# abcqmars/audio-visual-sepatation-in-visual-agnostic-situtation

Measured on AMD Instinct MI355X. Metric: mixtures/sec (train step, 2-src MUSIC shape), higher is better.
Workload: dtype f32; 1 GPU; full HIP path, AV train step: 2-source mix, batch 64/GPU (BASELINE configs[2] shape), 65535-sample waveforms -> HIP STFT 1022/256 -> 256x256 log-freq tiles, 3x224^2 frames/source, unet7+hidsep(sig)+resnet18dilated, BCE, SGD; f32 arithmetic; visual trunk on this library (no MIOpen kernel in the step); global_batch=64, parallelism=dp1

## Files before the change

### audio-visual-sepatation-in-visual-agnostic-situtation_amd/csrc/ops.hip

```cpp
#include "common.h"
#include "warp_coords.h"
#include <string.h>
#include <stdio.h>

__global__ __launch_bounds__(256) void channel_stats_kernel(const float* __restrict__ x, int N, int C, int HW,
                                                            double* __restrict__ stats) {
  const int c = blockIdx.x;
  const long long total = (long long)N * HW;
  const long long per = (total + gridDim.y - 1) / gridDim.y;
  const long long beg = per * blockIdx.y, end = min(total, beg + per);
  float s = 0.f, q = 0.f;
  double ds = 0.0, dq = 0.0;
  int cnt = 0;
  for (long long i = beg + threadIdx.x; i < end; i += 256) {
    int n = (int)(i / HW), hw = (int)(i % HW);
    float v = x[((long long)n * C + c) * HW + hw];
    s += v;
    q += v * v;
    if (++cnt == 64) { ds += s; dq += q; s = q = 0.f; cnt = 0; }
  }
  ds += s;
  dq += q;
  block_stats_add(ds, dq, c, C, stats);
}
// ... 115 lines not shown

enum { FORM_VEC4, FORM_SCALAR };
static bool plane_grid_ok(int N, int C, long long HW) {
  return N > 0 && N <= 65535 && C > 0 && C <= 65535 && HW > 0 && HW <= 0x7fffffffLL;
}
static GluePlan bn_bwd_apply_plan(int N, int C, long long HW) {
  if (!plane_grid_ok(N, C, HW)) return glue_refused();
  int gx = min(cdiv(HW, 1024), 64);
  return GluePlan{(HW & 3) == 0 ? FORM_VEC4 : FORM_SCALAR, dim3(gx, C, N)};
}
extern "C" int avsep_bn_bwd_apply(const float* dz, const float* y, const float* pqr, int32_t N, int32_t C, int32_t HW,
                                  float* dy, avsep_stream_t stream) {
  const GluePlan pl = bn_bwd_apply_plan(N, C, HW);
  if (!dz || !y || !pqr || !dy || pl.refused()) return AVSEP_ERR_ARG;
  hipLaunchKernelGGL(bn_bwd_apply_kernel, pl.grid, dim3(256), 0, (hipStream_t)stream, dz, y, pqr, C, HW, dy);
  AVSEP_LAUNCH_CHECK();
  return AVSEP_OK;
}

__global__ __launch_bounds__(256) void affine_act_kernel(const float* __restrict__ y, const float* __restrict__ scale,
                                                         const float* __restrict__ shift,
                                                         const float* __restrict__ res, const float* __restrict__ rscale,
                                                         const float* __restrict__ rshift, int act, int C, int HW,
                                                         float* __restrict__ z) {
  const int c = blockIdx.y, n = blockIdx.z;
  const float sc = scale ? scale[c] : 1.f, sh = shift ? shift[c] : 0.f;
  const float rs = rscale ? rscale[c] : 1.f, rh = rscale ? rshift[c] : 0.f;
  const long long base = ((long long)n * C + c) * HW;
  if ((HW & 3) == 0) {
    const float slope = act_slope(act);
// ... 344 lines not shown
      atomicAdd(&bstats1[cs], sh2[0] + sh2[1] + sh2[2] + sh2[3]);
      atomicAdd(&bstats1[a.C1 + cs], sh2[4] + sh2[5] + sh2[6] + sh2[7]);
    }
  }
}

static CatArgs make_cat(const avsep_cat_desc* d) {
  CatArgs a{};
  a.N = d->N; a.C0 = d->C0; a.C1 = d->C1; a.H = d->H; a.W = d->W; a.b0 = d->bcast0; a.b1 = d->bcast1;
  a.x0 = d->x0; a.x1 = d->x1; a.sc0 = d->scale0; a.sh0 = d->shift0; a.sc1 = d->scale1; a.sh1 = d->shift1;
  a.rh = (float)(d->H - 1) / (float)(2 * d->H - 1);
  a.rw = (float)(d->W - 1) / (float)(2 * d->W - 1);
  return a;
}
static bool cat_ok(const avsep_cat_desc* d) {
  return d && d->C0 > 0 && d->C1 >= 0 && d->x0 && (d->C1 == 0 || d->x1);
}

static int up2x_pair_lw(int H, int W, bool bcast) {
  if (bcast || W < 4 || W > 128 || (W & (W - 1)) || H < 2) return -1;
  int lw = 0;
  while ((2 << lw) < W) ++lw;
  return lw;
}
enum { UP2X_FWD_PAIR, UP2X_FWD_4, UP2X_FWD_GENERIC };
static GluePlan relu_up2x_fwd_plan(int N, int C, int H, int W, bool bcast) {
  if (N <= 0 || C <= 0 || H <= 0 || W <= 0) return glue_refused();
  const long long planes = (long long)N * C;
  if (planes > 0x7fffffffLL || 2 * H > 65535) return glue_refused();
  const int plw = up2x_pair_lw(H, W, bcast);
  if (plw >= 0 && planes <= 32768LL * 65535) {
// ... 135 lines not shown
    }
    const unsigned gy = (unsigned)(planes < 32768 ? planes : 32768), gz = (unsigned)cdiv(planes, gy);
    return GluePlan{UP2X_BWD_SWEEP, dim3(cdiv((long long)tp, 256), gy, gz), {plw, 0}};
  }
  if (C > 65535) return glue_refused();
  int tilesX = cdiv(W, UB_TW), tiles = tilesX * cdiv(H, UB_TH);
  int chunks = min(cdiv(4096, C * tiles), N);
  if (chunks < 1) chunks = 1;
  return GluePlan{UP2X_BWD_TILE, dim3(tiles, C, chunks), {tilesX, 0}};
}
extern "C" int avsep_relu_up2x_bwd(const avsep_cat_desc* d, const float* dout, float* g0, float* g1,
                                   const float* mean1, const float* invstd1, double* bstats1, int32_t acc0,
                                   avsep_stream_t stream) {
  if (!cat_ok(d) || !dout) return AVSEP_ERR_ARG;
  if (bstats1 && (!mean1 || !invstd1 || d->bcast1 || !g1)) return AVSEP_ERR_ARG;
  const GluePlan pl = relu_up2x_bwd_plan(d->N, d->C0 + d->C1, d->H, d->W, d->bcast0 || d->bcast1);
  if (pl.refused()) return AVSEP_ERR_ARG;
  CatArgs a = make_cat(d);
  switch (pl.form) {
    case UP2X_BWD_SWEEP_PLANES:
      hipLaunchKernelGGL(relu_up2x_bwd_sweep_kernel<true>, pl.grid, dim3(256), 0, (hipStream_t)stream, a, dout, g0, g1, mean1,
                         invstd1, bstats1, acc0, pl.arg[0], pl.arg[1]);
      break;
    case UP2X_BWD_SWEEP:
      hipLaunchKernelGGL(relu_up2x_bwd_sweep_kernel<false>, pl.grid, dim3(256), 0, (hipStream_t)stream, a, dout, g0, g1, mean1,
                         invstd1, bstats1, acc0, pl.arg[0], 0);
      break;
    case UP2X_BWD_TILE:
      hipLaunchKernelGGL(relu_up2x_bwd_kernel, pl.grid, dim3(256), 0, (hipStream_t)stream, a, dout, g0, g1, mean1, invstd1,
                         bstats1, acc0, pl.arg[0]);
// ... 728 lines not shown
    atomicAdd(&sums[r * 3 + 2], sh[8] + sh[9] + sh[10] + sh[11]);
  }
}
extern "C" int avsep_sdr_sums(const float* est, const float* ref, int32_t R, int32_t L, int64_t est_stride,
                              int64_t ref_stride, double* sums, avsep_stream_t stream) {
  if (!est || !ref || !sums || R <= 0 || R > 65535 || L <= 0) return AVSEP_ERR_ARG;
  hipLaunchKernelGGL(sdr_sums_kernel, dim3(min(cdiv(L, 2048), 64), R), dim3(256), 0, (hipStream_t)stream, est, ref, L,
                     (long long)est_stride, (long long)ref_stride, sums);
  AVSEP_LAUNCH_CHECK();
  return AVSEP_OK;
}

static const GluePlanRow ops_glue_rows[] = {
    {"channel_stats", {"chunks"}, [](int N, int C, int H, int W, int) { return channel_stats_plan(N, C, (long long)H * W); }},
    {"bn_bwd_apply", {"vec4", "scalar"}, [](int N, int C, int H, int W, int) { return bn_bwd_apply_plan(N, C, (long long)H * W); }},
    {"affine_act", {"vec4", "scalar"}, [](int N, int C, int H, int W, int) { return affine_act_plan(N, C, (long long)H * W); }},
    {"affine_act_bwd", {"v4", "v1"}, [](int N, int C, int H, int W, int) { return affine_act_bwd_plan(N, C, (long long)H * W); }},
    {"relu_up2x_fwd", {"pair", "fwd4", "generic"}, [](int N, int C, int H, int W, int aux) { return relu_up2x_fwd_plan(N, C, H, W, aux != 0); }},
    {"relu_up2x_bwd", {"sweep,planes", "sweep", "tile"}, [](int N, int C, int H, int W, int aux) { return relu_up2x_bwd_plan(N, C, H, W, aux != 0); }},
    {"maxpool_fwd", {"fwd4", "generic"}, [](int N, int C, int H, int W, int) { return maxpool_fwd_plan(C, (long long)N * C, H, W); }},
    {"maxpool_bwd", {"gather"}, [](int N, int C, int H, int W, int) { return maxpool_bwd_plan((long long)N * C, H, W); }},
    {"maxpool_bn_relu_bwd_stats", {"plane"}, [](int N, int C, int H, int W, int) { return maxpool_bn_relu_bwd_stats_plan(N, C, H, W); }},
    {"maxpool_bn_relu_bwd_apply", {"apply4", "pair", "apply1"}, [](int N, int C, int H, int W, int) { return maxpool_bn_relu_bwd_apply_plan(N, C, H, W); }},
    {"space_to_depth2", {"planes"}, [](int N, int C, int H, int W, int Cp) { return space_to_depth2_plan(N, C, H, W, Cp); }},
    {"temporal_mean_fwd", {"flat"}, [](int B, int C, int H, int W, int T) { return temporal_mean_plan(B, T, (long long)C * H * W, false); }},
    {"temporal_mean_bwd", {"flat"}, [](int B, int C, int H, int W, int T) { return temporal_mean_plan(B, T, (long long)C * H * W, true); }},
    {"sgd", {"flat"}, [](int N, int C, int H, int W, int) { return flat_plan((long long)N * C * ((long long)H * W), 16384); }},
};

extern "C" int avsep_glue_plan(const char* op, int32_t N, int32_t C, int32_t H, int32_t W, int32_t aux, char* form, size_t cap,
// ... 28 lines not shown
```

### audio-visual-sepatation-in-visual-agnostic-situtation_amd/kernels.py

```python
import ctypes as C
import os

import numpy as np
import torch

from . import lib
from .lib import ConvDesc, CatDesc, call, ptr


def _f32(shape, like):
    return torch.empty(shape, dtype=torch.float32, device=like.device)


FMT_F32, FMT_B16 = 0, 1


def is_b16(t):
    return t is not None and t.dtype == torch.bfloat16


def fmt_of(t):
    return FMT_B16 if is_b16(t) else FMT_F32


# ... 482 lines not shown
    N, Cc, H, W = dims(y)
    if to_b16_out and not is_b16(y) and not is_b16(dz) and b16_ok(Cc):
        dst = _b16((N, Cc, H, W), y)
        call("avsep_bn_bwd_apply_to_b16", ptr(dz), ptr(y), ptr(pqr), N, Cc, H * W, ptr(dst))
        return dst
    (dz,) = _same_fmt(y, dz)
    dst = torch.empty_like(y) if fresh else (dz if out is None else out)
    _drop_twin(dst)
    if is_b16(y):
        call("avsep_b16_bn_bwd_apply", ptr(dz), ptr(y), ptr(pqr), N, Cc, H * W, ptr(dst))
    else:
        call("avsep_bn_bwd_apply", ptr(dz), ptr(y), ptr(pqr), N, Cc, H * W, ptr(dst))
    return dst


def affine_act(y, scale, shift, residual, act, res_scale=None, res_shift=None):
    N, Cc, H, W = dims(y)
    z = torch.empty_like(y)
    (residual,) = _same_fmt(y, residual)
    if is_b16(y):
        call("avsep_b16_affine_act", ptr(y), ptr(scale), ptr(shift), ptr(residual), ptr(res_scale), ptr(res_shift), act, N, Cc,
             H * W, ptr(z))
    else:
        call("avsep_affine_act", ptr(y), ptr(scale), ptr(shift), ptr(residual), ptr(res_scale), ptr(res_shift), act, N, Cc,
             H * W, ptr(z))
    return z


def affine_act_bwd_(dz, y, scale, shift, residual, add, mean, invstd, act, bstats, res_scale=None, res_shift=None,
                    out=None, dz2=None, stats_only=False):
# ... 5 lines not shown
             ptr(res_shift), ptr(add), ptr(mean), ptr(invstd), act, N, Cc, H * W, None, ptr(bstats))
        return dz
    _drop_twin(dst)
    if is_b16(y):
        call("avsep_b16_affine_act_bwd", ptr(dz), ptr(dz2), ptr(y), ptr(scale), ptr(shift), ptr(residual), ptr(res_scale),
             ptr(res_shift), ptr(add), ptr(mean), ptr(invstd), act, N, Cc, H * W, ptr(dst), ptr(bstats))
    else:
        call("avsep_affine_act_bwd", ptr(dz), ptr(dz2), ptr(y), ptr(scale), ptr(shift), ptr(residual), ptr(res_scale), ptr(res_shift),
             ptr(add), ptr(mean), ptr(invstd), act, N, Cc, H * W, ptr(dst), ptr(bstats))
    return dst


class Cat:

    def __init__(self, x0, x1, sc0=None, sh0=None, sc1=None, sh1=None, bcast0=False, hw=None):
        self.b16 = (not bcast0 and x1 is not None and (is_b16(x0) or is_b16(x1)) and b16_ok(channels(x0))
                    and b16_ok(channels(x1)))
        if self.b16:
            x0, x1 = to_b16(x0), to_b16(x1)
        else:
            x0, x1 = to_f32(x0), to_f32(x1)
        N, C0 = (x0.shape[0], x0.shape[1]) if bcast0 else dims(x0)[:2]
        C1 = channels(x1) if x1 is not None else 0
        H, W = hw if hw is not None else (dims(x1)[2:] if x1 is not None else dims(x0)[2:])
        self.shape = (N, C0, C1, H, W)
        self.keep = (x0, x1, sc0, sh0, sc1, sh1)
        d = CatDesc()
        d.N, d.C0, d.C1, d.H, d.W, d.bcast0, d.bcast1 = N, C0, C1, H, W, int(bcast0), 0
        d.x0, d.x1 = ptr(x0), ptr(x1)
        d.scale0, d.shift0, d.scale1, d.shift1 = ptr(sc0), ptr(sh0), ptr(sc1), ptr(sh1)
        self.d, self.ref, self.like, self.bcast0 = d, C.byref(d), (x1 if x1 is not None else x0), bcast0

    def fwd(self):
        N, C0, C1, H, W = self.shape
        x0, x1, sc0, sh0, sc1, sh1 = self.keep
        if self.b16:
            out = _b16((N, C0 + C1, 2 * H, 2 * W), self.like)
# ... 4 lines not shown
        return out

    def bwd(self, dout, mean1=None, invstd1=None, bstats1=None, g0_acc=None):
        N, C0, C1, H, W = self.shape
        x0, x1, sc0, sh0, sc1, sh1 = self.keep
        if self.b16:
            dout = to_b16(dout)
            g0 = g0_acc if g0_acc is not None else _b16((N, C0, H, W), self.like)
            assert is_b16(g0), "accumulating into an fp32 skip gradient from a B16 decoder level"
            _drop_twin(g0)
            g1 = _b16((N, C1, H, W), self.like)
            call("avsep_b16_relu_up2x_bwd", ptr(x0), ptr(x1), ptr(sc0), ptr(sh0), ptr(sc1), ptr(sh1), N, C0, C1, H, W, ptr(dout),
                 ptr(g0), ptr(g1), ptr(mean1), ptr(invstd1), ptr(bstats1), int(g0_acc is not None))
            return g0, g1
        dout = to_f32(dout)
        g0 = g0_acc if g0_acc is not None else _f32((N, C0) if self.bcast0 else (N, C0, H, W), self.like)
        assert not is_b16(g0)
        _drop_twin(g0)
        g1 = _f32((N, C1, H, W), self.like) if C1 else None
        call("avsep_relu_up2x_bwd", self.ref, ptr(dout), ptr(g0), ptr(g1), ptr(mean1), ptr(invstd1),
             ptr(bstats1), int(g0_acc is not None))
        return g0, g1


def prepare(mag_mix, mags, log_freq, weighted, binary, fout=256):
    lib.require_gpu(mag_mix)
    S, B, _, Fin, T = mags.shape
    Fo = fout if log_freq else Fin
    mix_w, logm, weight = (_f32((B, 1, Fo, T), mag_mix) for _ in range(3))
    mags_w, gt = _f32((S, B, 1, Fo, T), mag_mix), _f32((S, B, 1, Fo, T), mag_mix)
    call("avsep_prepare", ptr(mag_mix), ptr(mags), S, B, Fin, T, Fo, int(bool(log_freq)), int(bool(weighted)),
         int(bool(binary)), ptr(mix_w), ptr(mags_w), ptr(logm), ptr(weight), ptr(gt))
    return mix_w, mags_w, logm, weight, gt
# ... 785 lines not shown
```

### audio-visual-sepatation-in-visual-agnostic-situtation_amd/lib.py

```python
import ctypes as C
import os

import torch

_HERE = os.path.dirname(os.path.abspath(__file__))
LIB_PATH = os.path.join(_HERE, "libavsep_gfx950.so")

ACT_NONE, ACT_RELU, ACT_LRELU02, ACT_SIGMOID, ACT_TANH, ACT_SOFTMAX2 = range(6)
ACT_BY_NAME = {"no": ACT_NONE, "relu": ACT_RELU, "sigmoid": ACT_SIGMOID, "tanh": ACT_TANH,
               "softmax": ACT_SOFTMAX2}
LOSS_BY_NAME = {"bce": 0, "l1": 1, "l2": 2}
ATT_BY_NAME = {"cos": 0, "sig": 1}
ALGO_NO = {"winograd": 1, "winograd_wgrad": 2, "flat": 4, "misc_patch": 8, "bf16_kernels": 16, "smallci_wgrad": 32, "winograd4": 64}


class AvsepError(RuntimeError):
    pass


class ConvDesc(C.Structure):
    _fields_ = [(n, C.c_int32) for n in
                "N Cin H W Cout Ho Wo KH KW stride pad dil C0 act0 act1 up2x prec plan_n xfmt yfmt dyfmt dxfmt algo tune".split()] + \
               [(n, C.c_void_p) for n in "x0 x1 scale0 shift0 scale1 shift1".split()]

# ... 56 lines not shown
    "avsep_conv_kernel_name": (C.c_char_p, [_CD, _I, _I]),
    "avsep_conv_kernel_variant": (C.c_int, [_CD, _I, _I, C.c_char_p, _Z]),
    "avsep_space_to_depth2": (C.c_int, [_P, _I, _I, _I, _I, _I, _P, _P]),
    "avsep_maxpool_bn_relu_bwd_stats": (C.c_int, [_P, _P, _P, _P, _P, _P, _P, _I, _I, _I, _I, _P, _P]),
    "avsep_maxpool_bn_relu_bwd_apply": (C.c_int, [_P, _P, _P, _P, _P, _P, _I, _I, _I, _I, _P, _P]),
    "avsep_attmodel_infer_fwd": (C.c_int, [_P, _P, _I, _I, _I, _I, _I, _P, _P, _P, _P]),
    "avsep_attmodel_infer_bwd": (C.c_int, [_P, _P, _P, _P, _P, _P, _I, _I, _I, _I, _I, _P, _P, _P]),
    "avsep_conv2d_dgrad_up2x_workspace_bytes": (_Z, [_CD]),
    "avsep_conv2d_dgrad_up2x": (C.c_int, [_CD, _P, _P, _P, _P, _P, _P, _P, _I, _P, _Z, _P]),
    "avsep_conv2d_wgrad_workspace_bytes": (_Z, [_CD]),
    "avsep_conv2d_wgrad": (C.c_int, [_CD, _P, _P, _P, _P, _Z, _P]),
    "avsep_channel_stats": (C.c_int, [_P, _I, _I, _I, _P, _P]),
    "avsep_bn_finalize": (C.c_int, [_P, _D, _P, _P, _P, _P, _F, _F, _I, _I, _P, _P, _P, _P, _P, _I, _P]),
    "avsep_bn_bwd_coeffs": (C.c_int, [_P, _D, _P, _P, _P, _I, _P, _P, _P, _P]),
    "avsep_bn_bwd_apply": (C.c_int, [_P, _P, _P, _I, _I, _I, _P, _P]),
    "avsep_affine_act": (C.c_int, [_P, _P, _P, _P, _P, _P, _I, _I, _I, _I, _P, _P]),
    "avsep_affine_act_bwd": (C.c_int, [_P, _P, _P, _P, _P, _P, _P, _P, _P, _P, _P, _I, _I, _I, _I, _P, _P, _P]),
    "avsep_relu_up2x_fwd": (C.c_int, [_KD, _P, _P]),
    "avsep_relu_up2x_bwd": (C.c_int, [_KD, _P, _P, _P, _P, _P, _P, _I, _P]),
    "avsep_prepare": (C.c_int, [_P, _P, _I, _I, _I, _I, _I, _I, _I, _I, _P, _P, _P, _P, _P, _P]),
    "avsep_warp": (C.c_int, [_P, _I, _I, _I, _I, _I, _I, _P, _P]),
    "avsep_window_prepare": (C.c_int, [_P, _I, _I, _P, _I, _I, _I, _P, _P, _P]),
    "avsep_window_agreement": (C.c_int, [_P, _P, _I, _I, _I, _I, _P, _P]),
    "avsep_mask_stitch": (C.c_int, [_P, _P, _P, _P, _I, _I, _I, _I, _I, _I, _I, _I, _F, _P, _P, _P]),
    "avsep_window_reduce": (C.c_int, [_P, _P, _I, _I, C.c_int64, _I, _P, _P]),
    "avsep_mwf_workspace_bytes": (_Z, [_I, _I, _I, _I]),
    "avsep_mwf_cov": (C.c_int, [_P, _P, _I, _I, _I, _I, _I, _P, _P, _Z, _P]),
    "avsep_mwf_apply": (C.c_int, [_P, _P, _P, _P, _I, _I, _I, _I, _F, _P, _P, _P]),
    "avsep_mwf_tv_workspace_bytes": (_Z, [_I, _I, _I, _I, _I]),
    "avsep_mwf_cov_tv": (C.c_int, [_P, _P, _I, _I, _I, _I, _I, _I, _P, _P, _Z, _P]),
# ... 128 lines not shown
```

### audio-visual-sepatation-in-visual-agnostic-situtation_amd/models/audio_net.py

```python
import os

import torch
import torch.nn as nn

from .. import kernels as K
from .. import lib
from ..lib import ACT_LRELU02, ACT_NONE, ACT_RELU
from . import fusion_net

BN_EPS, BN_MOMENTUM = 1e-5, 0.1


class _Slots(nn.Module):
    def put(self, idx, mod):
        self.add_module(str(idx), mod)
        return mod

    def at(self, idx):
        return getattr(self, str(idx))


class Conv2dParams(nn.Module):

    def __init__(self, cin, cout, k, bias):
# ... 36 lines not shown
            object.__setattr__(self, name, value)
        else:
            super().__setattr__(name, value)


class Unet(nn.Module):
    def __init__(self, fc_dim=64, num_downs=5, ngf=64, use_dropout=False, fusion_type="con_motion",
                 att_type="cos", fuse_upsample=False, extra_size=None):
        super().__init__()
        if use_dropout:
            raise NotImplementedError("use_dropout is never enabled by the reference builders")
        self.extra_size = extra_size
        self.fusion_type, self.att_type = fusion_type, att_type
        self.fuse_upsample = fuse_upsample
        self.fuse_head = True
        if extra_size is None:
            self.fusion = fusion_net.get_fusion_net(fusion_type)(att_type=att_type)
            self.fusion.num_src = fc_dim if 2 < fc_dim <= 4 else 2
            lvl = _Level(ngf * 8, ngf * 8, ngf * 8, ngf * 16, "inner", None)
        else:
            self.fusion = None
            lvl = _Level(ngf * 8, ngf * 8 + 2 * extra_size, ngf * 8, ngf * 8, "inner", None)
        for _ in range(num_downs - 5):
            lvl = _Level(ngf * 8, ngf * 8, ngf * 8, ngf * 16, "mid", lvl)
        lvl = _Level(ngf * 4, ngf * 8, ngf * 4, ngf * 16, "mid", lvl)
        lvl = _Level(ngf * 2, ngf * 4, ngf * 2, ngf * 8, "mid", lvl)
        lvl = _Level(ngf, ngf * 2, ngf, ngf * 4, "mid", lvl)
        lvl = _Level(fc_dim, ngf, 1, ngf * 2, "outer", lvl)
        self.bn0 = BatchNorm2dParams(1)
        self.unet_block = lvl
# ... 157 lines not shown
    E["bn0"] = _bn_run(net.bn0, st0, B * H * W, training, x, repeat)
    src, aff, act = x, E["bn0"], ACT_NONE
    E["dconv"], E["yd"], E["dbn"] = [], [], []
    for l in lv:
        w = l.down_conv.weight.detach()
        cv = K.Conv(src, w.shape[0], 4, 2, 1, sc0=aff[0] if aff is not None else None,
                    sh0=aff[1] if aff is not None else None, act0=act)
        st = K.zeros_stats(w.shape[0], x) if (l.down_bn is not None and training) else None
        y = cv.fwd(cv.pack(w, 0), None, st)
        bn = _bn_run(l.down_bn, st, K.per_channel(y), training, x, repeat) if l.down_bn is not None else None
        E["dconv"].append(cv); E["yd"].append(y); E["dbn"].append(bn)
        src, aff, act = y, bn, ACT_LRELU02
    return E


def _decode(net, E, vs, draws, training):
    lv, x = E["lv"], E["x"]
    L = len(lv)
    ybot = K.to_f32(E["yd"][-1])
    extra = fus = feat_vec = None
    if net.extra_size is None:
        fus = net.fusion.run_forward(ybot, vs, draws)
        feat_vec = fus["feat"]
    else:
        e2 = 2 * net.extra_size
        extra, ybot = ybot[:, :e2].contiguous(), ybot[:, e2:].contiguous()
    D = {"fus": fus, "ybot": ybot, "extra": extra, "vs": vs,
         "uconv": [None] * L, "yu": [None] * L, "ubn": [None] * L, "cat": [None] * L}
    for i in range(L - 1, -1, -1):
        l = lv[i]
        w = l.up_conv.weight.detach()
        if i == L - 1:
            cat = K.Cat(feat_vec, ybot, bcast0=True) if feat_vec is not None else K.Cat(ybot, None)
            fused = False
        else:
            dbn, ubn = E["dbn"][i], D["ubn"][i + 1]
            cat = K.Cat(E["yd"][i], D["yu"][i + 1], sc0=dbn[0] if dbn is not None else None,
                        sh0=dbn[1] if dbn is not None else None, sc1=ubn[0], sh1=ubn[1])
            fused = net.fuse_upsample
        cv = None
        if i < L - 1:
            cv = K.Conv(cat.keep[0], w.shape[0], 3, 1, 1, x1=cat.keep[1], sc0=cat.keep[2], sh0=cat.keep[3],
                        act0=ACT_RELU, sc1=cat.keep[4], sh1=cat.keep[5], act1=ACT_RELU, up2x=True)
            cv.head = cv.head_applicable() and net.fuse_head
            fused = fused or cv.head
        if not fused:
            cv = K.Conv(cat.fwd(), w.shape[0], 3, 1, 1)
            cv.head = False
        st = K.zeros_stats(w.shape[0], x) if (l.up_bn is not None and training) else None
        bias = l.up_conv.bias.detach() if l.up_conv.bias is not None else None
        y = cv.fwd(cv.pack(w, 0), bias, st, out_b16=False if (i == 1 and net.fuse_head) else None)
        bn = _bn_run(l.up_bn, st, K.per_channel(y), training, x) if l.up_bn is not None else None
        D["uconv"][i], D["yu"][i], D["ubn"][i], D["cat"][i] = cv, y, bn, cat
    return D


def _decode_bwd(net, E, D, dlogits, dsecond, has_vis, grads, Gd, order=None):
    lv, x = E["lv"], E["x"]

    def gd_sync(i, when):
        if order is None:
            return
        mode, evs = order
        if mode == "record" and when == "after":
            evs[i] = torch.cuda.Event()
            evs[i].record()
        elif mode == "wait" and when == "before" and evs[i] is not None:
            torch.cuda.current_stream().wait_event(evs[i])
    L = len(lv)
    g = dlogits.contiguous()
    dfeat = dbot = None
    for i in range(L):
        l, cv, cat = lv[i], D["uconv"][i], D["cat"][i]
        w = l.up_conv.weight.detach()
        grads.wgrad(cv, l.up_conv.weight, g, l.up_conv.bias)
        if cv.head:
            ubn = D["ubn"][i + 1]
            bst = K.zeros_stats(ubn.shape[1], x)
            gd_sync(i, "before")
            Gd[i], dz = cv.dgrad_up2x(w, g, mean1=ubn[2], invstd1=ubn[3], bstats1=bst, g0_acc=Gd[i])
            gd_sync(i, "after")
            yu = D["yu"][i + 1]
            g = K.bn_bwd_apply_(dz, yu, _bn_back(grads, lv[i + 1].up_bn, ubn, bst, K.per_channel(yu)),
                                to_b16_out=K.want_b16(K.channels(yu)))
            continue
        dU = cv.dgrad(cv.pack(w, 1), g, out_b16=cat.b16)
        if i == L - 1:
            if net.extra_size is None:
                dfeat, dbot = cat.bwd(dU)
            else:
                dxb, _ = cat.bwd(dU)
                dbot = torch.cat([dsecond.to(dxb.dtype).contiguous(), dxb], 1)
        else:
            ubn = D["ubn"][i + 1]
            bst = K.zeros_stats(ubn.shape[1], x)
            gd_sync(i, "before")
            Gd[i], dz = cat.bwd(dU, mean1=ubn[2], invstd1=ubn[3], bstats1=bst, g0_acc=Gd[i])
            gd_sync(i, "after")
            yu = D["yu"][i + 1]
            pqr = _bn_back(grads, lv[i + 1].up_bn, ubn, bst, K.per_channel(yu))
            g = K.bn_bwd_apply_(dz, yu, pqr)
        del dU
    dvs = []
    if net.extra_size is None:
        dvs = net.fusion.run_backward(D["ybot"], D["vs"], D["fus"], dfeat, dbot, None, dsecond if has_vis else None)
    return dbot, dvs


def _encode_bwd(net, E, dbot, Gd, grads):
    lv, x = E["lv"], E["x"]
    g = dbot
    for i in range(len(lv) - 1, -1, -1):
        l, cv = lv[i], E["dconv"][i]
        w = l.down_conv.weight.detach()
        grads.wgrad(cv, l.down_conv.weight, g)
        dS = cv.dgrad(cv.pack(w, 1), g, out_b16=K.is_b16(E["yd"][i - 1]) if i > 0 else False)
# ... 15 lines not shown
def _outputs(net, D, x):
    logits = D["yu"][0]
    if net.extra_size is not None:
        return logits, D["extra"], x.new_zeros(())
    if D["vs"]:
        return logits, D["fus"]["match_part"].mean(), D["fus"]["att_maps"]
    return logits, x.new_zeros(()), x.new_zeros(())


class _UnetFn(torch.autograd.Function):
    @staticmethod
    def forward(ctx, net, draws, nv, x, *rest):
        vs, training = list(rest[:nv]), net.training
        _release_deferred(net)
        E = _encode(net, x, training)
        D = _decode(net, E, vs, draws, training)
        ctx.E, ctx.D, ctx.net, ctx.nv, ctx.training = E, D, net, nv, training
        out = _outputs(net, D, x)
        if net.extra_size is None:
            ctx.mark_non_differentiable(out[2])
        return out

    @staticmethod
    def backward(ctx, dlogits, dsecond, _datt):
        if not ctx.training:
            raise lib.AvsepError("backward through the U-Net needs train mode (batch statistics)")
        net, E, D = ctx.net, ctx.E, ctx.D
        grads, Gd = ParamGrads(net), [None] * len(E["lv"])
        dbot, dvs = _decode_bwd(net, E, D, dlogits, dsecond, bool(ctx.nv), grads, Gd)
        _encode_bwd(net, E, dbot, Gd, grads)
# ... 18 lines not shown
        return None
    s = net.__dict__.get("_pair_side")
    if s is None:
        s = torch.cuda.Stream()
        object.__setattr__(net, "_pair_side", s)
    return s


class _UnetPairFn(torch.autograd.Function):

    @staticmethod
    def forward(ctx, net, nv, x, *rest):
        training = net.training
        _release_deferred(net)
        E = _encode(net, x, training, repeat=2)
        hook = net.__dict__.pop("_before_decode", None)
        if hook is not None:
            hook()
        side = _pair_stream(net, x)
        if side is None:
            Da = _decode(net, E, list(rest[:nv]), None, training)
            Db = _decode(net, E, list(rest[nv:2 * nv]), None, training)
        else:
            main, fork = torch.cuda.current_stream(), torch.cuda.Event()
            fork.record()
            with K.fork_streams():
                Da = _decode(net, E, list(rest[:nv]), None, training)
                side.wait_event(fork)
                with torch.cuda.stream(side):
                    Db = _decode(net, E, list(rest[nv:2 * nv]), None, training)
# ... 1 lines not shown
        ctx.E, ctx.Da, ctx.Db, ctx.net, ctx.training = E, Da, Db, net, training
        oa, ob = _outputs(net, Da, x), _outputs(net, Db, x)
        if side is not None:
            for t in ob:
                t.record_stream(torch.cuda.current_stream())
        ctx.mark_non_differentiable(oa[2], ob[2])
        return (*oa, *ob)

    @staticmethod
    def backward(ctx, dla, dma, _a, dlb, dmb, _b):
        if not ctx.training:
            raise lib.AvsepError("backward through the U-Net needs train mode (batch statistics)")
        net, E = ctx.net, ctx.E
        grads, Gd = ParamGrads(net), [None] * len(E["lv"])
        side = _pair_stream(net, E["x"]) if grads.sink is not None else None
        if side is None:
            dbot_a, dva = _decode_bwd(net, E, ctx.Da, dla, dma, True, grads, Gd)
            dbot_b, dvb = _decode_bwd(net, E, ctx.Db, dlb, dmb, True, grads, Gd)
        else:
            main, fork, evs = torch.cuda.current_stream(), torch.cuda.Event(), [None] * len(E["lv"])
            fork.record()
            dbot_a, dva = _decode_bwd(net, E, ctx.Da, dla, dma, True, grads, Gd, order=("record", evs))
            done_a = torch.cuda.Event()
            done_a.record()
            side.wait_event(done_a if grads.second else fork)
            with torch.cuda.stream(side):
                dbot_b, dvb = _decode_bwd(net, E, ctx.Db, dlb, dmb, True, grads, Gd, order=("wait", evs))
                done_b = torch.cuda.Event()
                done_b.record()
                side.wait_event(done_a)
                grads.fold_second()
            if not getattr(net, "encoder_bwd_on_side", _ENC_SIDE):
                main.wait_stream(side)
                for t in [dbot_b, *dvb]:
                    if t is not None:
                        t.record_stream(main)
                _encode_bwd(net, E, dbot_a.add_(dbot_b), Gd, grads)
                ctx.E = ctx.Da = ctx.Db = None
                return (None, None, None, *dva, *dvb, *grads.finish(net.param_list(), "sound"))
            with torch.cuda.stream(side):
                _encode_bwd(net, E, dbot_b.add_(dbot_a), Gd, grads)
                pg = grads.finish(net.param_list(), "sound")
            main.wait_event(done_b)
            for t in dvb:
                if t is not None:
                    t.record_stream(main)
            if any(g is not None for g in pg):
                main.wait_stream(side)
            object.__setattr__(net, "_pair_deferred", (E, ctx.Da, ctx.Db, Gd, dbot_a, dbot_b))
            grads.sink.at_end_of_backward(lambda: _release_deferred(net))
            ctx.E = ctx.Da = ctx.Db = None
            return (None, None, None, *dva, *dvb, *pg)
        _encode_bwd(net, E, dbot_a.add_(dbot_b), Gd, grads)
        ctx.E = ctx.Da = ctx.Db = None
        return (None, None, None, *dva, *dvb, *grads.finish(net.param_list(), "sound"))
```

### include/avsep.h

```cpp
#ifndef AVSEP_H
#define AVSEP_H
#include <stddef.h>
#include <stdint.h>

#ifdef __cplusplus
extern "C" {
#endif

#define AVSEP_OK 0
#define AVSEP_ERR_ARG (-1)
#define AVSEP_ERR_LAUNCH (-2)
#define AVSEP_ERR_WORKSPACE (-3)

#define AVSEP_ACT_NONE 0
#define AVSEP_ACT_RELU 1
#define AVSEP_ACT_LRELU02 2
#define AVSEP_ACT_SIGMOID 3
#define AVSEP_ACT_TANH 4
#define AVSEP_ACT_SOFTMAX2 5

#define AVSEP_PREC_F32 0
#define AVSEP_PREC_BF16 1

#define AVSEP_FMT_F32 0
// ... 82 lines not shown
int avsep_attmodel_infer_bwd(const float* a, const float* mix, const float* maps_raw, const float* dctx,
                             const float* dmaps, const float* dmatch, int32_t B, int32_t S, int32_t K, int32_t HW,
                             int32_t att, float* da, float* dmix, avsep_stream_t stream);

int avsep_channel_stats(const float* x, int32_t N, int32_t C, int32_t HW, double* stats,
                        avsep_stream_t stream);
int avsep_bn_finalize(const double* stats, double count, const float* gamma, const float* beta,
                      float* running_mean, float* running_var, float momentum, float eps,
                      int32_t C, int32_t training, float* scale, float* shift, float* mean,
                      float* invstd, int64_t* num_batches_tracked, int32_t updates, avsep_stream_t stream);
int avsep_bn_bwd_coeffs(const double* bstats, double count, const float* gamma, const float* mean,
                        const float* invstd, int32_t C, float* dgamma, float* dbeta, float* pqr,
                        avsep_stream_t stream);
int avsep_bn_bwd_apply(const float* dz, const float* y, const float* pqr, int32_t N, int32_t C,
                       int32_t HW, float* dy, avsep_stream_t stream);
int avsep_affine_act(const float* y, const float* scale, const float* shift, const float* residual,
                     const float* res_scale, const float* res_shift, int32_t act, int32_t N, int32_t C,
                     int32_t HW, float* z, avsep_stream_t stream);
int avsep_affine_act_bwd(const float* dz, const float* dz2, const float* y, const float* scale, const float* shift,
                         const float* residual, const float* res_scale, const float* res_shift,
                         const float* add, const float* mean, const float* invstd, int32_t act,
                         int32_t N, int32_t C, int32_t HW, float* dz_pre, double* bstats,
                         avsep_stream_t stream);

typedef struct avsep_cat_desc {
  int32_t N, C0, C1, H, W;
  int32_t bcast0, bcast1;
  const float* x0;
  const float* x1;
  const float* scale0;
// ... 304 lines not shown
```

Baseline: 875.2 mixtures/s.

## Share skip-half of decoder up-conv across the two source decodes

In the paired decode, the U-Net up-conv input is a concat of an encoder skip (identical for both sources) and a source-specific inner branch. The forward now materialises the skip half once and runs the conv with split inputs. An optional backward path runs the skip-half wgrad/dgrad once on the summed cotangent of both decodes, using a fused BN-backward-apply-plus-sum kernel and a weight-grad assembly kernel. The intent is to avoid computing the skip-half dgrad and wgrad twice. It adds cross-stream event coordination, and the backward sharing is off by default (share_skip_backward=False). The forward split also drops the fused up2x/head path at those levels.

```diff
diff --git a/audio-visual-sepatation-in-visual-agnostic-situtation_amd/csrc/ops.hip b/audio-visual-sepatation-in-visual-agnostic-situtation_amd/csrc/ops.hip
--- a/audio-visual-sepatation-in-visual-agnostic-situtation_amd/csrc/ops.hip
+++ b/audio-visual-sepatation-in-visual-agnostic-situtation_amd/csrc/ops.hip
@@ -153,6 +153,71 @@
   const GluePlan pl = bn_bwd_apply_plan(N, C, HW);
   if (!dz || !y || !pqr || !dy || pl.refused()) return AVSEP_ERR_ARG;
   hipLaunchKernelGGL(bn_bwd_apply_kernel, pl.grid, dim3(256), 0, (hipStream_t)stream, dz, y, pqr, C, HW, dy);
+  AVSEP_LAUNCH_CHECK();
+  return AVSEP_OK;
+}
+
+__global__ __launch_bounds__(256) void bn_bwd_apply_sum_kernel(const float* __restrict__ dz, const float* __restrict__ y,
+                                                               const float* __restrict__ pqr, const float* __restrict__ other,
+                                                               int C, int HW, float* __restrict__ dy, float* __restrict__ sum) {
+  const int c = blockIdx.y, n = blockIdx.z;
+  const float p = pqr[c], q = pqr[C + c], r = pqr[2 * C + c];
+  const long long base = ((long long)n * C + c) * HW;
+  if ((HW & 3) == 0) {
+    const float4* dz4 = reinterpret_cast<const float4*>(dz + base);
+    const float4* y4 = reinterpret_cast<const float4*>(y + base);
+    const float4* t4 = reinterpret_cast<const float4*>(other + base);
+    float4* o4 = reinterpret_cast<float4*>(dy + base);
+    float4* s4 = reinterpret_cast<float4*>(sum + base);
+    for (int i = blockIdx.x * 256 + threadIdx.x; i < HW / 4; i += gridDim.x * 256) {
+      float4 a = dz4[i], b = y4[i], t = t4[i], o, s;
+      o.x = fmaf(p, a.x, fmaf(q, b.x, r));
+      o.y = fmaf(p, a.y, fmaf(q, b.y, r));
+      o.z = fmaf(p, a.z, fmaf(q, b.z, r));
+      o.w = fmaf(p, a.w, fmaf(q, b.w, r));
+      s.x = o.x + t.x; s.y = o.y + t.y; s.z = o.z + t.z; s.w = o.w + t.w;
+      o4[i] = o;
+      s4[i] = s;
+    }
+  } else {
+    for (int i = blockIdx.x * 256 + threadIdx.x; i < HW; i += gridDim.x * 256) {
+      const float o = fmaf(p, dz[base + i], fmaf(q, y[base + i], r));
+      dy[base + i] = o;
+      sum[base + i] = o + other[base + i];
+    }
+  }
+}
+extern "C" int avsep_bn_bwd_apply_sum(const float* dz, const float* y, const float* pqr, const float* other, int32_t N,
+                                      int32_t C, int32_t HW, float* dy, float* sum, avsep_stream_t stream) {
+  const GluePlan pl = bn_bwd_apply_plan(N, C, HW);
+  if (!dz || !y || !pqr || !other || !dy || !sum || sum == dy || sum == dz || pl.refused()) return AVSEP_ERR_ARG;
+  hipLaunchKernelGGL(bn_bwd_apply_sum_kernel, pl.grid, dim3(256), 0, (hipStream_t)stream, dz, y, pqr, other, C, HW, dy, sum);
+  AVSEP_LAUNCH_CHECK();
+  return AVSEP_OK;
+}
+
+__global__ __launch_bounds__(256) void wgrad_assemble_kernel(const float* __restrict__ skip, const float* __restrict__ inner_a,
+                                                             const float* __restrict__ inner_b, int n0, int n1, long long total,
+                                                             float* __restrict__ dw) {
+  const int row = n0 + n1;
+  for (long long i = (long long)blockIdx.x * 256 + threadIdx.x; i < total; i += (long long)gridDim.x * 256) {
+    const long long co = i / row;
+    const int j = (int)(i - co * row);
+    dw[i] = j < n0 ? skip[co * n0 + j] : inner_a[co * n1 + (j - n0)] + inner_b[co * n1 + (j - n0)];
+  }
+}
+static GluePlan wgrad_assemble_plan(int Cout, int C0, int C1, long long T) {
+  if (Cout <= 0 || C0 <= 0 || C1 <= 0 || T <= 0 || T > 65536) return glue_refused();
+  const long long row = ((long long)C0 + C1) * T;
+  if (row > 0x7fffffffLL || row * Cout > (1LL << 36)) return glue_refused();
+  return GluePlan{0, dim3(min(cdiv(row * Cout, 256), 16384))};
+}
+extern "C" int avsep_wgrad_assemble(const float* skip, const float* inner_a, const float* inner_b, int32_t Cout, int32_t C0,
+                                    int32_t C1, int32_t taps, float* dw, avsep_stream_t stream) {
+  const GluePlan pl = wgrad_assemble_plan(Cout, C0, C1, taps);
+  if (!skip || !inner_a || !inner_b || !dw || pl.refused()) return AVSEP_ERR_ARG;
+  hipLaunchKernelGGL(wgrad_assemble_kernel, pl.grid, dim3(256), 0, (hipStream_t)stream, skip, inner_a, inner_b, C0 * taps,
+                     C1 * taps, ((long long)C0 + C1) * taps * Cout, dw);
   AVSEP_LAUNCH_CHECK();
   return AVSEP_OK;
 }
@@ -527,7 +592,8 @@
   return a;
 }
 static bool cat_ok(const avsep_cat_desc* d) {
-  return d && d->C0 > 0 && d->C1 >= 0 && d->x0 && (d->C1 == 0 || d->x1);
+  return d && d->C0 >= 0 && d->C1 >= 0 && (long long)d->C0 + d->C1 > 0 && (d->C0 == 0 || d->x0) && (d->C1 == 0 || d->x1) &&
+         !(d->C0 == 0 && d->bcast0) && !(d->C1 == 0 && d->bcast1);
 }
 
 static int up2x_pair_lw(int H, int W, bool bcast) {
@@ -693,6 +759,7 @@
                                    avsep_stream_t stream) {
   if (!cat_ok(d) || !dout) return AVSEP_ERR_ARG;
   if (bstats1 && (!mean1 || !invstd1 || d->bcast1 || !g1)) return AVSEP_ERR_ARG;
+  if (d->C0 == 0 && !g1) return AVSEP_ERR_ARG;
   const GluePlan pl = relu_up2x_bwd_plan(d->N, d->C0 + d->C1, d->H, d->W, d->bcast0 || d->bcast1);
   if (pl.refused()) return AVSEP_ERR_ARG;
   CatArgs a = make_cat(d);
@@ -1451,6 +1518,8 @@
 static const GluePlanRow ops_glue_rows[] = {
     {"channel_stats", {"chunks"}, [](int N, int C, int H, int W, int) { return channel_stats_plan(N, C, (long long)H * W); }},
     {"bn_bwd_apply", {"vec4", "scalar"}, [](int N, int C, int H, int W, int) { return bn_bwd_apply_plan(N, C, (long long)H * W); }},
+    {"bn_bwd_apply_sum", {"vec4", "scalar"}, [](int N, int C, int H, int W, int) { return bn_bwd_apply_plan(N, C, (long long)H * W); }},
+    {"wgrad_assemble", {"flat"}, [](int Cout, int C0, int KH, int KW, int C1) { return wgrad_assemble_plan(Cout, C0, C1, (long long)KH * KW); }},
     {"affine_act", {"vec4", "scalar"}, [](int N, int C, int H, int W, int) { return affine_act_plan(N, C, (long long)H * W); }},
     {"affine_act_bwd", {"v4", "v1"}, [](int N, int C, int H, int W, int) { return affine_act_bwd_plan(N, C, (long long)H * W); }},
     {"relu_up2x_fwd", {"pair", "fwd4", "generic"}, [](int N, int C, int H, int W, int aux) { return relu_up2x_fwd_plan(N, C, H, W, aux != 0); }},
diff --git a/audio-visual-sepatation-in-visual-agnostic-situtation_amd/kernels.py b/audio-visual-sepatation-in-visual-agnostic-situtation_amd/kernels.py
--- a/audio-visual-sepatation-in-visual-agnostic-situtation_amd/kernels.py
+++ b/audio-visual-sepatation-in-visual-agnostic-situtation_amd/kernels.py
@@ -520,6 +520,59 @@
     return dst
 
 
+def bn_bwd_apply_sum_(dz, y, pqr, other):
+    if any(is_b16(t) or not t.is_contiguous() or tuple(t.shape) != tuple(y.shape) for t in (dz, y, other)):
+        raise lib.AvsepError("bn_bwd_apply_sum_ takes dense fp32 tensors of one shape")
+    N, Cc, H, W = y.shape
+    total = torch.empty_like(y)
+    _drop_twin(dz)
+    call("avsep_bn_bwd_apply_sum", ptr(dz), ptr(y), ptr(pqr), ptr(other), N, Cc, H * W, ptr(dz), ptr(total))
+    return dz, total
+
+
+def wgrad_assemble(skip, inner_a, inner_b, out=None):
+    Cout, C0, KH, KW = skip.shape
+    C1 = inner_a.shape[1]
+    shape = (Cout, C0 + C1, KH, KW)
+    if tuple(inner_a.shape) != (Cout, C1, KH, KW) or inner_b.shape != inner_a.shape or \
+            not all(t.is_contiguous() and t.dtype == torch.float32 for t in (skip, inner_a, inner_b)):
+        raise lib.AvsepError("wgrad_assemble takes dense fp32 OIHW halves of one conv")
+    if out is not None and (tuple(out.shape) != shape or not out.is_contiguous() or out.dtype != torch.float32):
+        raise lib.AvsepError("wgrad_assemble destination must be a dense fp32 OIHW tensor")
+    dw = out if out is not None else _f32(shape, skip)
+    call("avsep_wgrad_assemble", ptr(skip), ptr(inner_a), ptr(inner_b), Cout, C0, C1, KH * KW, ptr(dw))
+    return dw
+
+
+def split_up_conv_served(like, N, C0, C1, H, W, cout):
+    if _precision != 0 or C0 != C1 or C0 <= 0:
+        return False
+    key = (N, C0, C1, H, W, cout, plan_batch_scale, algo_mask, conv_tune)
+    hit = _split_memo.get(key)
+    if hit is not None:
+        return hit
+
+    def names(cin, c0):
+        d = ConvDesc()
+        d.N, d.Cin, d.H, d.W, d.Cout, d.Ho, d.Wo = N, cin, H, W, cout, H, W
+        d.KH, d.KW, d.stride, d.pad, d.dil, d.C0 = 3, 3, 1, 1, 1, c0
+        d.plan_n = N * plan_batch_scale if plan_batch_scale != 1 else 0
+        d.algo, d.tune = algo_mask, conv_tune
+        d.x0 = d.x1 = ptr(like)
+        if c0 == cin:
+            d.x1 = None
+        L = lib.load()
+        return [L.avsep_conv_kernel_name(C.byref(d), m, s).decode() for m, s in ((0, 1), (0, 0), (1, 0), (2, 0))]
+    dense, pair, skip, inner = names(C0 + C1, C0 + C1), names(C0 + C1, C0), names(C0, C0), names(C1, C1)
+    ok = "invalid" not in dense and pair == dense and skip[2:] == dense[2:] and inner[2:] == dense[2:]
+    ok = ok and dense[2] != "wino_kernel"
+    _split_memo[key] = ok
+    return ok
+
+
+_split_memo = {}
+
+
 def affine_act(y, scale, shift, residual, act, res_scale=None, res_shift=None):
     N, Cc, H, W = dims(y)
     z = torch.empty_like(y)
@@ -555,13 +608,16 @@
 class Cat:
 
     def __init__(self, x0, x1, sc0=None, sh0=None, sc1=None, sh1=None, bcast0=False, hw=None):
-        self.b16 = (not bcast0 and x1 is not None and (is_b16(x0) or is_b16(x1)) and b16_ok(channels(x0))
+        self.b16 = (not bcast0 and x0 is not None and x1 is not None and (is_b16(x0) or is_b16(x1)) and b16_ok(channels(x0))
                     and b16_ok(channels(x1)))
         if self.b16:
             x0, x1 = to_b16(x0), to_b16(x1)
         else:
             x0, x1 = to_f32(x0), to_f32(x1)
-        N, C0 = (x0.shape[0], x0.shape[1]) if bcast0 else dims(x0)[:2]
+        if x0 is None:
+            N, C0 = x1.shape[0], 0
+        else:
+            N, C0 = (x0.shape[0], x0.shape[1]) if bcast0 else dims(x0)[:2]
         C1 = channels(x1) if x1 is not None else 0
         H, W = hw if hw is not None else (dims(x1)[2:] if x1 is not None else dims(x0)[2:])
         self.shape = (N, C0, C1, H, W)
@@ -596,9 +652,12 @@
                  ptr(g0), ptr(g1), ptr(mean1), ptr(invstd1), ptr(bstats1), int(g0_acc is not None))
             return g0, g1
         dout = to_f32(dout)
-        g0 = g0_acc if g0_acc is not None else _f32((N, C0) if self.bcast0 else (N, C0, H, W), self.like)
-        assert not is_b16(g0)
-        _drop_twin(g0)
+        if C0 == 0:
+            g0 = None
+        else:
+            g0 = g0_acc if g0_acc is not None else _f32((N, C0) if self.bcast0 else (N, C0, H, W), self.like)
+            assert not is_b16(g0)
+            _drop_twin(g0)
         g1 = _f32((N, C1, H, W), self.like) if C1 else None
         call("avsep_relu_up2x_bwd", self.ref, ptr(dout), ptr(g0), ptr(g1), ptr(mean1), ptr(invstd1),
              ptr(bstats1), int(g0_acc is not None))
diff --git a/audio-visual-sepatation-in-visual-agnostic-situtation_amd/lib.py b/audio-visual-sepatation-in-visual-agnostic-situtation_amd/lib.py
--- a/audio-visual-sepatation-in-visual-agnostic-situtation_amd/lib.py
+++ b/audio-visual-sepatation-in-visual-agnostic-situtation_amd/lib.py
@@ -94,6 +94,8 @@
     "avsep_bn_finalize": (C.c_int, [_P, _D, _P, _P, _P, _P, _F, _F, _I, _I, _P, _P, _P, _P, _P, _I, _P]),
     "avsep_bn_bwd_coeffs": (C.c_int, [_P, _D, _P, _P, _P, _I, _P, _P, _P, _P]),
     "avsep_bn_bwd_apply": (C.c_int, [_P, _P, _P, _I, _I, _I, _P, _P]),
+    "avsep_bn_bwd_apply_sum": (C.c_int, [_P, _P, _P, _P, _I, _I, _I, _P, _P, _P]),
+    "avsep_wgrad_assemble": (C.c_int, [_P, _P, _P, _I, _I, _I, _I, _P, _P]),
     "avsep_affine_act": (C.c_int, [_P, _P, _P, _P, _P, _P, _I, _I, _I, _I, _P, _P]),
     "avsep_affine_act_bwd": (C.c_int, [_P, _P, _P, _P, _P, _P, _P, _P, _P, _P, _P, _I, _I, _I, _I, _P, _P, _P]),
     "avsep_relu_up2x_fwd": (C.c_int, [_KD, _P, _P]),
diff --git a/audio-visual-sepatation-in-visual-agnostic-situtation_amd/models/audio_net.py b/audio-visual-sepatation-in-visual-agnostic-situtation_amd/models/audio_net.py
--- a/audio-visual-sepatation-in-visual-agnostic-situtation_amd/models/audio_net.py
+++ b/audio-visual-sepatation-in-visual-agnostic-situtation_amd/models/audio_net.py
@@ -74,6 +74,8 @@
         self.fusion_type, self.att_type = fusion_type, att_type
         self.fuse_upsample = fuse_upsample
         self.fuse_head = True
+        self.share_skip = True
+        self.share_skip_backward = False
         if extra_size is None:
             self.fusion = fusion_net.get_fusion_net(fusion_type)(att_type=att_type)
             self.fusion.num_src = fc_dim if 2 < fc_dim <= 4 else 2
@@ -261,9 +263,27 @@
     return E
 
 
+def _skip_halves(net, E):
+    L = len(E["lv"])
+    E["skip_hi"], E["skip_cat"] = [None] * L, [None] * L
+    net.split_levels = []
+    if not getattr(net, "share_skip", True) or net.fuse_upsample or K.get_precision() != "f32":
+        return
+    for i in range(1, L - 1):
+        yd, w = E["yd"][i], E["lv"][i].up_conv.weight
+        N, C0, H, W = K.dims(yd)
+        if K.is_b16(yd) or w.shape[0] <= 4 or not K.split_up_conv_served(yd, N, C0, w.shape[1] - C0, 2 * H, 2 * W, w.shape[0]):
+            continue
+        dbn = E["dbn"][i]
+        cat = K.Cat(yd, None, sc0=dbn[0] if dbn is not None else None, sh0=dbn[1] if dbn is not None else None)
+        E["skip_cat"][i], E["skip_hi"][i] = cat, cat.fwd()
+    net.split_levels = [i for i in range(L) if E["skip_hi"][i] is not None]
+
+
 def _decode(net, E, vs, draws, training):
     lv, x = E["lv"], E["x"]
     L = len(lv)
+    skip_hi = E.get("skip_hi") or [None] * L
     ybot = K.to_f32(E["yd"][-1])
     extra = fus = feat_vec = None
     if net.extra_size is None:
@@ -286,7 +306,11 @@
                         sh0=dbn[1] if dbn is not None else None, sc1=ubn[0], sh1=ubn[1])
             fused = net.fuse_upsample
         cv = None
-        if i < L - 1:
+        if skip_hi[i] is not None:
+            inner = K.Cat(None, D["yu"][i + 1], sc1=ubn[0], sh1=ubn[1])
+            cv = K.Conv(skip_hi[i], w.shape[0], 3, 1, 1, x1=inner.fwd())
+            cv.head, cv.inner_cat, fused = False, inner, True
+        elif i < L - 1:
             cv = K.Conv(cat.keep[0], w.shape[0], 3, 1, 1, x1=cat.keep[1], sc0=cat.keep[2], sh0=cat.keep[3],
                         act0=ACT_RELU, sc1=cat.keep[4], sh1=cat.keep[5], act1=ACT_RELU, up2x=True)
             cv.head = cv.head_applicable() and net.fuse_head
@@ -302,8 +326,44 @@
     return D
 
 
-def _decode_bwd(net, E, D, dlogits, dsecond, has_vis, grads, Gd, order=None):
+class _SkipShare:
+
+    def __init__(self, E, forked):
+        self.levels = [i for i, t in enumerate(E["skip_hi"]) if t is not None]
+        L = len(E["lv"])
+        self.role, self.forked = "A", forked
+        self.g_a, self.g_s, self.ev = [None] * L, [None] * L, [None] * L
+        self.dw = [{} for _ in range(L)]
+        self.w = [None] * L
+        for i in self.levels:
+            w, C0 = E["lv"][i].up_conv.weight.detach(), K.channels(E["yd"][i])
+            self.w[i] = (w[:, :C0].contiguous(), w[:, C0:].contiguous())
+
+    def cotangent(self, i, dz, yu, pqr):
+        if self.role == "A":
+            g = self.g_a[i] = K.bn_bwd_apply_(dz, yu, pqr)
+            if self.forked:
+                self.ev[i] = torch.cuda.Event()
+                self.ev[i].record()
+            return g
+        if self.ev[i] is not None:
+            torch.cuda.current_stream().wait_event(self.ev[i])
+            self.g_a[i].record_stream(torch.cuda.current_stream())
+        g, self.g_s[i] = K.bn_bwd_apply_sum_(dz, yu, pqr, self.g_a[i])
+        return g
+
+    def finish(self, E, grads):
+        for i in self.levels:
+            p, h = E["lv"][i].up_conv.weight, self.dw[i]
+            if self.forked:
+                h["a"].record_stream(torch.cuda.current_stream())
+            out = grads.dest(p)
+            grads.add(p, K.wgrad_assemble(h["s"], h["a"], h["b"], out), out)
+
+
+def _decode_bwd(net, E, D, dlogits, dsecond, has_vis, grads, Gd, order=None, share=None):
     lv, x = E["lv"], E["x"]
+    split = E.get("skip_hi") or [None] * len(lv)
 
     def gd_sync(i, when):
         if order is None:
@@ -314,12 +374,37 @@
             evs[i].record()
         elif mode == "wait" and when == "before" and evs[i] is not None:
             torch.cuda.current_stream().wait_event(evs[i])
+
+    def next_g(i, dz, bst, to_b16=False):
+        ubn, yu = D["ubn"][i + 1], D["yu"][i + 1]
+        pqr = _bn_back(grads, lv[i + 1].up_bn, ubn, bst, K.per_channel(yu))
+        if share is not None and split[i + 1] is not None:
+            return share.cotangent(i + 1, dz, yu, pqr)
+        return K.bn_bwd_apply_(dz, yu, pqr, to_b16_out=to_b16)
     L = len(lv)
     g = dlogits.contiguous()
     dfeat = dbot = None
     for i in range(L):
         l, cv, cat = lv[i], D["uconv"][i], D["cat"][i]
         w = l.up_conv.weight.detach()
+        if share is not None and split[i] is not None:
+            ubn, cout = D["ubn"][i + 1], w.shape[0]
+            w_skip, w_inner = share.w[i]
+            half = K.Conv(cv.keep[1], cout, 3, 1, 1)
+            share.dw[i]["a" if share.role == "A" else "b"] = half.wgrad(g)[0]
+            dU = half.dgrad(half.pack(w_inner, 1), g, out_b16=False)
+            bst = K.zeros_stats(ubn.shape[1], x)
+            _, dz = cv.inner_cat.bwd(dU, mean1=ubn[2], invstd1=ubn[3], bstats1=bst)
+            del dU
+            g_s, g = share.g_s[i], next_g(i, dz, bst)
+            if share.role == "B":
+                half = K.Conv(split[i], cout, 3, 1, 1)
+                share.dw[i]["s"] = half.wgrad(g_s)[0]
+                dU = half.dgrad(half.pack(w_skip, 1), g_s, out_b16=False)
+                Gd[i], _ = E["skip_cat"][i].bwd(dU)
+                share.g_s[i] = share.g_a[i] = None
+                del dU, g_s
+            continue
         grads.wgrad(cv, l.up_conv.weight, g, l.up_conv.bias)
         if cv.head:
             ubn = D["ubn"][i + 1]
@@ -327,9 +412,7 @@
             gd_sync(i, "before")
             Gd[i], dz = cv.dgrad_up2x(w, g, mean1=ubn[2], invstd1=ubn[3], bstats1=bst, g0_acc=Gd[i])
             gd_sync(i, "after")
-            yu = D["yu"][i + 1]
-            g = K.bn_bwd_apply_(dz, yu, _bn_back(grads, lv[i + 1].up_bn, ubn, bst, K.per_channel(yu)),
-                                to_b16_out=K.want_b16(K.channels(yu)))
+            g = next_g(i, dz, bst, to_b16=K.want_b16(K.channels(D["yu"][i + 1])))
             continue
         dU = cv.dgrad(cv.pack(w, 1), g, out_b16=cat.b16)
         if i == L - 1:
@@ -344,9 +427,7 @@
             gd_sync(i, "before")
             Gd[i], dz = cat.bwd(dU, mean1=ubn[2], invstd1=ubn[3], bstats1=bst, g0_acc=Gd[i])
             gd_sync(i, "after")
-            yu = D["yu"][i + 1]
-            pqr = _bn_back(grads, lv[i + 1].up_bn, ubn, bst, K.per_channel(yu))
-            g = K.bn_bwd_apply_(dz, yu, pqr)
+            g = next_g(i, dz, bst)
         del dU
     dvs = []
     if net.extra_size is None:
@@ -392,6 +473,7 @@
         vs, training = list(rest[:nv]), net.training
         _release_deferred(net)
         E = _encode(net, x, training)
+        _skip_halves(net, E)
         D = _decode(net, E, vs, draws, training)
         ctx.E, ctx.D, ctx.net, ctx.nv, ctx.training = E, D, net, nv, training
         out = _outputs(net, D, x)
@@ -440,6 +522,7 @@
         training = net.training
         _release_deferred(net)
         E = _encode(net, x, training, repeat=2)
+        _skip_halves(net, E)
         hook = net.__dict__.pop("_before_decode", None)
         if hook is not None:
             hook()
@@ -471,25 +554,36 @@
         net, E = ctx.net, ctx.E
         grads, Gd = ParamGrads(net), [None] * len(E["lv"])
         side = _pair_stream(net, E["x"]) if grads.sink is not None else None
+        share = None
+        if getattr(net, "share_skip_backward", False) and any(t is not None for t in E["skip_hi"]):
+            share = _SkipShare(E, side is not None)
         if side is None:
-            dbot_a, dva = _decode_bwd(net, E, ctx.Da, dla, dma, True, grads, Gd)
-            dbot_b, dvb = _decode_bwd(net, E, ctx.Db, dlb, dmb, True, grads, Gd)
+            dbot_a, dva = _decode_bwd(net, E, ctx.Da, dla, dma, True, grads, Gd, share=share)
+            if share is not None:
+                share.role = "B"
+            dbot_b, dvb = _decode_bwd(net, E, ctx.Db, dlb, dmb, True, grads, Gd, share=share)
+            if share is not None:
+                share.finish(E, grads)
         else:
             main, fork, evs = torch.cuda.current_stream(), torch.cuda.Event(), [None] * len(E["lv"])
             fork.record()
-            dbot_a, dva = _decode_bwd(net, E, ctx.Da, dla, dma, True, grads, Gd, order=("record", evs))
+            dbot_a, dva = _decode_bwd(net, E, ctx.Da, dla, dma, True, grads, Gd, order=("record", evs), share=share)
+            if share is not None:
+                share.role = "B"
             done_a = torch.cuda.Event()
             done_a.record()
             side.wait_event(done_a if grads.second else fork)
             with torch.cuda.stream(side):
-                dbot_b, dvb = _decode_bwd(net, E, ctx.Db, dlb, dmb, True, grads, Gd, order=("wait", evs))
+                dbot_b, dvb = _decode_bwd(net, E, ctx.Db, dlb, dmb, True, grads, Gd, order=("wait", evs), share=share)
                 done_b = torch.cuda.Event()
                 done_b.record()
                 side.wait_event(done_a)
+                if share is not None:
+                    share.finish(E, grads)
                 grads.fold_second()
             if not getattr(net, "encoder_bwd_on_side", _ENC_SIDE):
                 main.wait_stream(side)
-                for t in [dbot_b, *dvb]:
+                for t in [dbot_b, *dvb, *(Gd[i] for i in (share.levels if share is not None else ()))]:
                     if t is not None:
                         t.record_stream(main)
                 _encode_bwd(net, E, dbot_a.add_(dbot_b), Gd, grads)
@@ -504,7 +598,7 @@
                     t.record_stream(main)
             if any(g is not None for g in pg):
                 main.wait_stream(side)
-            object.__setattr__(net, "_pair_deferred", (E, ctx.Da, ctx.Db, Gd, dbot_a, dbot_b))
+            object.__setattr__(net, "_pair_deferred", (E, ctx.Da, ctx.Db, Gd, dbot_a, dbot_b, share))
             grads.sink.at_end_of_backward(lambda: _release_deferred(net))
             ctx.E = ctx.Da = ctx.Db = None
             return (None, None, None, *dva, *dvb, *pg)
diff --git a/include/avsep.h b/include/avsep.h
--- a/include/avsep.h
+++ b/include/avsep.h
@@ -120,6 +120,10 @@
                         avsep_stream_t stream);
 int avsep_bn_bwd_apply(const float* dz, const float* y, const float* pqr, int32_t N, int32_t C,
                        int32_t HW, float* dy, avsep_stream_t stream);
+int avsep_bn_bwd_apply_sum(const float* dz, const float* y, const float* pqr, const float* other, int32_t N,
+                           int32_t C, int32_t HW, float* dy, float* sum, avsep_stream_t stream);
+int avsep_wgrad_assemble(const float* skip, const float* inner_a, const float* inner_b, int32_t Cout, int32_t C0,
+                         int32_t C1, int32_t taps, float* dw, avsep_stream_t stream);
 int avsep_affine_act(const float* y, const float* scale, const float* shift, const float* residual,
                      const float* res_scale, const float* res_shift, int32_t act, int32_t N, int32_t C,
                      int32_t HW, float* z, avsep_stream_t stream);
```

New measurement: 878.8 mixtures/s (median of 6 runs). No clear change (+0.4%).
